# bywmm/RE-GNN

Measured on AMD Instinct MI355X. Metric: aggregated edges/sec per GPU (REGCN fwd+bwd, hidden=64); % HBM roofline, higher is better.
Workload: dtype fp32; 1 GPU; mag/regnn_ns.py REGCN neighbour-sampled train step: device sampler 512 papers/rank x fan-out [25, 20], group_input, 2x REGCNConv (hidden 64, mean, relation table, LN, ReLU, dropout 0.5), out_lin 349, nll, backward, Adam; mag_like(scale=10.0) replicated per rank; nodes=19397430, edges=422220140, relations=11, hidden=64, batch_per_rank=512, global_batch=512, parallelism=dp1, lookahead=16, hip_graph=True, engine=fused regnn_nsm_step

## Files before the change

### __graft_entry__.py

```python
import os
import sys

ROOT = os.path.dirname(os.path.abspath(__file__))
PKG = os.path.join(ROOT, "re-gnn_amd")
for _p in (ROOT, PKG):
    if _p not in sys.path:
        sys.path.insert(0, _p)


def build():
    from regnn_hip import build as b
    b.build()
    ob = os.path.join(ROOT, "oracle", "build_oracle.py")
    if os.path.exists(ob):
        import runpy
        runpy.run_path(ob, run_name="__main__")
    import layer
    import dgl
    from regnn_hip import _lib
    assert _lib.ABI_VERSION == 46


def smoke():
    import numpy as np
    import torch
    import torch.nn.functional as F

    build()
    sys.path.insert(0, os.path.join(ROOT, "tests"))
    import _golden as G
    from oracle import regnn_oracle as O
    import dgl
    from regnn_hip import nets

    d = G.load("model_regcn2")
    m = d["meta"]
    g = dgl.DGLGraph((d["g_src"], d["g_dst"]), num_nodes=int(d["g_N"])).to("cuda:0")
    net = nets.REGCN(g, int(d["g_R"]), m["alpha"], 64, 64, m["n_classes"], 2, F.elu, 0.0, m["dims"])
    P = G.sub(d, "p_", np.float32)
    with torch.no_grad():
        for n, p in net.named_parameters():
            p.copy_(torch.from_numpy(P[n]))
    net = net.to("cuda:0").eval()
    feats = [torch.from_numpy(d[f"feat{i}"]).to("cuda:0") for i in range(len(m["dims"]))]
    e_feat = torch.from_numpy(d["g_rel"]).to("cuda:0")
    logits, _ = net(feats, e_feat)
    logits.backward(torch.from_numpy(d["gout"]).to("cuda:0"))
    torch.cuda.synchronize()
    og = O.Graph(d["g_src"], d["g_dst"], int(d["g_N"]))
    ref_logits, _, ref_grads = O.regcn_model(
        og, [d[f"feat{i}"].astype(np.float64) for i in range(len(m["dims"]))], d["g_rel"],
        G.sub(d, "p_"), 2, m["alpha"], d["gout"].astype(np.float64))
    ok, err = G.close(logits.detach().cpu().numpy(), ref_logits, 1e-5)
# ... 10 lines not shown
```

### include/regnn_hip.h

```cpp
#ifndef REGNN_HIP_H
#define REGNN_HIP_H
#include <stdint.h>

#ifdef __cplusplus
extern "C" {
#endif

typedef struct ihipStream_t* hipStream_t;

enum { REGNN_OK = 0, REGNN_EINVAL = 1, REGNN_EUNSUPPORTED = 2, REGNN_ELAUNCH = 3 };
enum { REGNN_F32 = 0, REGNN_BF16 = 1 };
enum { REGNN_SELF_PRESCALED = 0x100 };

int regnn_abi_version(void);

int64_t regnn_tune(int32_t key, int64_t value);

int64_t regnn_slab_rows(int64_t n_seg, int32_t n_chunk);

int regnn_degree(const int32_t* ptr, const uint8_t* rel, const float* rel_table, int64_t n_seg,
                 float power, int32_t split, const int32_t* long_ids, int32_t n_long,
                 const int32_t* long_cnt, int32_t n_rel, float* deg, float* norm,
                 hipStream_t stream);

// ... 243 lines not shown
                   int32_t world, int64_t* state, int32_t* n_id, int32_t* sizes,
                   int64_t* stamp_src, hipStream_t stream);

#define REGNN_CSC_PIECE 1024
#define REGNN_CSC_LONG_CAP (32768 / 17 + 1)
#define REGNN_CSC_LONG_NPIECE (REGNN_CSC_LONG_CAP + 1)
#define REGNN_CSC_LONG_TAB (((REGNN_CSC_LONG_NPIECE + 1) + 3) / 4 * 4)
#define REGNN_CSC_LONG_MAXPIECE (32768 / REGNN_CSC_PIECE + REGNN_CSC_LONG_CAP)
#define REGNN_CSC_LONG_INTS (REGNN_CSC_LONG_TAB + 4 * REGNN_CSC_LONG_MAXPIECE)
int regnn_ns_hop(const int32_t* ptr, const int32_t* idx, const uint8_t* etype,
                 const int32_t* ntype, int32_t num_edge_types, int32_t k, int32_t hop,
                 int64_t* state, int32_t* sizes, int32_t* n_id, int32_t cap_dst,
                 uint64_t* g2l, uint64_t* first, int32_t* samp, int32_t* spos, int32_t* scnt,
                 int32_t* gsrc, uint8_t* flag, int32_t* tiles, uint64_t* status,
                 int32_t* blk_ptr, int32_t* blk_idx, uint8_t* blk_rel, int32_t* blk_pos,
                 int32_t* blk_row, float* inv, const int64_t* local, int32_t* edge_type,
                 int64_t* edge_off, int32_t meta_only, int32_t* csc_cnt, int32_t* csc_ptr,
                 int32_t* csc_ent, int32_t* csc_long, int32_t strided, hipStream_t stream);

typedef struct regnn_ns_csc_job {
    int32_t hop;
    int32_t cap_e;
    const int32_t* gsrc;
    const uint64_t* g2l;
    int32_t* blk_idx;
    const int32_t* blk_row;
    const uint8_t* blk_rel;
    int32_t* csc_cnt;
    int32_t* tiles;
    int32_t* csc_ptr;
    int32_t* csc_ent;
    int32_t* csc_long;
} regnn_ns_csc_job;
int regnn_ns_hop_typed_sums(const int32_t* ptr, const int32_t* idx, const uint8_t* etype,
                            const int32_t* ntype, int32_t num_edge_types, int32_t k, int32_t hop,
                            int64_t* state, int32_t* sizes, const int32_t* n_id, int32_t cap_dst,
                            int32_t* scnt, uint8_t* blk_rel, float* inv, const int64_t* local,
                            int32_t* edge_type, int64_t* edge_off, const float* const* tables,
                            int32_t n_types, int32_t K, float* s_agg, float* s_w, float* u_self,
                            int32_t* u_rel, const regnn_ns_csc_job* csc, hipStream_t stream);

int regnn_ns_spmm_bwd(const int32_t* ptr, const int32_t* idx, const uint8_t* rel,
                      const float* rel_table, const float* out_scale, const float* g,
                      const float* x, float* gx, float* slab, int32_t n_rel, int64_t n_rows,
                      int32_t F, hipStream_t stream);

int64_t regnn_ns_csc_hub_work_floats(int32_t F);
int regnn_ns_spmm_bwd_csc(const int32_t* csc_ptr, const int32_t* csc_ent, const int32_t* csc_long,
                          const float* rel_table, const float* out_scale, const float* g,
                          const float* x, float* gx, float* slab, int32_t n_rel,
                          const int32_t* sizes, int32_t size_idx, int64_t cap_rows, int32_t F,
                          int32_t slab_rows, float* hub_work, hipStream_t stream);

int regnn_ns_typed_agg(const int32_t* ptr, const int32_t* idx, const uint8_t* rel,
                       const float* rel_table, const int32_t* n_id, const int32_t* ntype,
                       const int64_t* local, const int32_t* e_type, const int64_t* e_off,
                       const float* const* tables, int32_t n_types, int32_t K, int64_t n_rows,
                       float* S, float* wsum, int64_t ld_s, int64_t ld_w, hipStream_t stream);

int regnn_ns_spmm_strided_fwd(const int32_t* live, const int32_t* cnt, int32_t stride,
                              const int32_t* idx, const uint8_t* rel, const float* rel_table,
                              const float* inv, const float* bias, const float* x, float* y,
                              int64_t n_rows, int32_t F, hipStream_t stream);

int regnn_ns_slot_agg(const int32_t* sizes, int32_t hop, const float* U, const float* cnt,
                      const float* x_self, const int32_t* u_rel, const float* rel_table,
                      int32_t n_et, int32_t n_types, int32_t K, int64_t cap, float* out,
                      int64_t ld, hipStream_t stream);
int regnn_ns_slot_agg_bwd(const int32_t* sizes, int32_t hop, const float* U, const float* cnt,
                          const float* x_self, const int32_t* u_rel, const float* g, int64_t ld,
                          int32_t n_et, int32_t n_types, int32_t K, float* slab, int32_t n_rel,
                          int32_t slab_rows, hipStream_t stream);

// ... 155 lines not shown
```

### re-gnn_amd/csrc/re_ns.hip

```cpp
#include "regnn_common.h"

#include <cstdlib>

namespace regnn {

constexpr int kNsTile = 1024;

__device__ __forceinline__ uint64_t mix64(uint64_t x) {
    x ^= x >> 30;
    x *= 0xBF58476D1CE4E5B9ull;
    x ^= x >> 27;
    x *= 0x94D049BB133111EBull;
    x ^= x >> 31;
    return x;
}

__device__ __forceinline__ uint64_t ns_hop_seed(const int64_t* state, int hop) {
    const uint64_t base = uint64_t(state[0]), epoch = uint64_t(state[1]),
                   batch = uint64_t(state[3]);
    return mix64(base ^ mix64((epoch << 40) ^ (batch << 8) ^ uint64_t(hop)));
}

__device__ __forceinline__ uint32_t ns_stamp(const int64_t* state, int hop) {
    return uint32_t(uint64_t(state[4]) * 8u + uint64_t(hop) + 1u);
// ... 755 lines not shown
        for (uint32_t spins = 0; spins < (1u << 26) && !seen; ++spins) {
            seen = uint32_t(__hip_atomic_load(ctl + 1, __ATOMIC_RELAXED,
                                              __HIP_MEMORY_SCOPE_AGENT)) == stamp;
            if (!seen) __builtin_amdgcn_s_sleep(1);
        }
        if (!seen) {
            __hip_atomic_store(ctl + 2, 1, __ATOMIC_RELAXED, __HIP_MEMORY_SCOPE_AGENT);
            ok = 0;
        }
        __builtin_amdgcn_fence(__ATOMIC_ACQUIRE, "agent");
        asm volatile("s_waitcnt vmcnt(0)" ::: "memory");
    }
    __syncthreads();
    if (lid >= 0 && ok) J.csc_ent[J.csc_ptr[lid] + rank] = ent;
}

inline int csc_blocks(int64_t cap_e) { return int((cap_e + kCscScanT - 1) / kCscScanT); }

__global__ void __launch_bounds__(kCscScanT)
ns_resolve_csc_kernel(NsCscJob J, const int32_t* __restrict__ sizes,
                      const int64_t* __restrict__ state) {
    csc_resolve_place<16>(J, sizes, state, blockIdx.x, gridDim.x);
}

struct NsSumArgs {
    const int32_t* ptr; const int32_t* idx; const uint8_t* etype; const int32_t* ntype;
    const int64_t* local; int n_et;
    const int32_t* n_id; int32_t* sizes; int hop; int cap; int k;
    int64_t* state;
    int32_t* scnt; uint8_t* blk_rel; float* inv; int32_t* e_type; int64_t* e_off;
    const float* xt[8]; int T;
    float* s_agg; float* s_w; float* u_self; int32_t* u_rel;
    NsCscJob csc; int csc_blocks;
};

template <int NT>
__device__ __forceinline__ const float* pick_tab(const NsSumArgs& A, int t) {
    const float* r = A.xt[0];
#pragma unroll
    for (int q = 1; q < NT; ++q)
        if (t == q) r = A.xt[q];
    return r;
}

constexpr int kNsSumK = 128;
#ifndef REGNN_NS_SUM_UN32
#define REGNN_NS_SUM_UN32 11
#endif
template <int G>
constexpr int ns_sum_un() { return G == 32 ? REGNN_NS_SUM_UN32 : 11; }
constexpr int kNsSumOcc = REGNN_NS_SUM_UN32 > 11 ? 3 : 4;
constexpr int kNsSumWaves = 4;

template <int G, int NT>
__global__ void __launch_bounds__(64 * kNsSumWaves, kNsSumOcc)
ns_sample_sums_kernel(NsSumArgs A) {
    if (int(blockIdx.x) < A.csc_blocks) {
        csc_resolve_place<4>(A.csc, A.sizes, A.state, blockIdx.x, A.csc_blocks);
        return;
    }
    const int bid = blockIdx.x - A.csc_blocks, nbk = gridDim.x - A.csc_blocks;
    constexpr int K = kNsSumK;
    constexpr int kNsSumUN = ns_sum_un<G>();
    constexpr int TPW = 64 / G;
    constexpr int H = G == 64 ? 2 : 1;
    __shared__ int wsum[kNsSumWaves * TPW];
    const int wl = threadIdx.x & 63, wv = threadIdx.x >> 6;
    const int lane = wl % G, tl = wv * TPW + wl / G;
    const uint64_t gmask = G == 64 ? ~0ull : (0xFFFFFFFFull << (wl & 32));
    const int n = A.sizes[A.hop];
    const int k = A.k, S = k + 1;
    int etot = 0;
    for (int ib = bid * (kNsSumWaves * TPW); ib < A.cap; ib += nbk * (kNsSumWaves * TPW)) {
    const int i = ib + tl;
    const int64_t base = int64_t(i) * S;
    int cnt = -1;
    if (i < A.cap && i >= n) {
        if (lane == 0) {
            A.scnt[i] = 0;
            A.inv[i] = 1.f;
        }
    } else if (i < n) {
        const uint64_t seed = ns_hop_seed(A.state, A.hop);
        const int t = A.n_id[i];
        const int b = A.ptr[t], d = A.ptr[t + 1] - b;
        cnt = d < k ? d : k;
        int slot = lane < d ? lane : -1, rank = lane;
        int src = lane;
        if (d > k) {
            slot = -1;
            const int jl = d - k + lane;
            const int my_pos = lane < k ? int((uint64_t(ns_hash(seed, uint64_t(t), uint64_t(jl))) *
                                               uint64_t(jl + 1)) >> 32) : 0;
            for (int q = 0; q < k; ++q) {
                const int pos = __shfl(my_pos, q, G);
                const bool seen = (__ballot(slot == pos) & gmask) != 0;
                if (lane == q) slot = seen ? d - k + q : pos;
            }
            rank = 0;
            for (int m = 0; m < k; ++m) {
                const int other = __shfl(slot, m, G);
                rank += (lane < k && other < slot) ? 1 : 0;
            }
            for (int m = 0; m < k; ++m)
                if (__shfl(rank, m, G) == lane) src = m;
        }
        int my_t = 0, my_lo = 0, my_r = 0;
        if (lane < cnt) {
            const int p = b + slot;
            const int u = A.idx[p];
            const int64_t bp = base + rank;
            my_r = A.etype[p];
            my_t = A.ntype[u];
            const int64_t lo = A.local[u];
            my_lo = int(lo);
            A.blk_rel[bp] = uint8_t(my_r);
            A.e_type[bp] = my_t;
            A.e_off[bp] = lo;
        }
        int st = __shfl(my_t, src, G), sr = __shfl(my_r, src, G), slo = __shfl(my_lo, src, G);
        if (lane == cnt) {
            const int64_t bp = base + cnt;
            st = A.ntype[t];
            sr = A.n_et + st;
            const int64_t lo = A.local[t];
            slo = int(lo);
            A.blk_rel[bp] = uint8_t(sr);
            A.e_type[bp] = st;
            A.e_off[bp] = lo;
        }
        if (lane == 0) {
            A.scnt[i] = cnt;
            A.inv[i] = 1.f / float(cnt + 1);
        }
        const int h = lane >> 5, l = lane & 31;
        const int ne = cnt + 1;
        float4 racc[NT];
        float ws[NT];
        int rt[NT];
#pragma unroll
        for (int tt = 0; tt < NT; ++tt) {
            racc[tt] = make_float4(0.f, 0.f, 0.f, 0.f);
            ws[tt] = 0.f;
            rt[tt] = -1;
        }
        float4 xs = make_float4(0.f, 0.f, 0.f, 0.f);
        int rs = -1;
        for (int j0 = 0; j0 < ne; j0 += H * kNsSumUN) {
            float4 x[kNsSumUN];
#pragma unroll
            for (int u = 0; u < kNsSumUN; ++u) {
                const int j = j0 + H * u + h;
                const int jj = j < ne ? j : ne - 1;
                const int tj = __shfl(st, jj, G);
                const int64_t lo = __shfl(slo, jj, G);
                x[u] = *reinterpret_cast<const float4*>(pick_tab<NT>(A, tj) + lo * K + 4 * l);
            }
#pragma unroll
            for (int u = 0; u < kNsSumUN; ++u) {
                const int j = j0 + H * u + h;
                const int jj = j < ne ? j : ne - 1;
                const int tj = __shfl(st, jj, G), rj = __shfl(sr, jj, G);
// ... 721 lines not shown
                       edge_type, edge_off, lean, csc_cnt, int(cap_e));
    REGNN_LAUNCH_CHECK();
    const int64_t slots = int64_t(cap_dst) * k;
    hipLaunchKernelGGL(ns_place_kernel, dim3(unsigned((slots + kBlock - 1) / kBlock)),
                       dim3(kBlock), 0, stream, samp, spos, scnt, sizes, hop, cap_dst, k, state,
                       etype, g2l, first, blk_ptr, blk_rel, blk_pos, blk_row, gsrc, ntype, local, edge_type,
                       edge_off, lean);
    REGNN_LAUNCH_CHECK();
    if (lean) return REGNN_OK;
    hipLaunchKernelGGL(ns_flags_kernel, dim3(n_tiles), dim3(kBlock), 0, stream, gsrc, sizes, hop,
                       state, g2l, first, flag, tiles, n_tiles, 0);
    REGNN_LAUNCH_CHECK();
    hipLaunchKernelGGL(ns_finish_kernel, dim3(n_tiles), dim3(kBlock), 0, stream, gsrc, sizes, hop,
                       state, flag, tiles, g2l, n_id, 0);
    REGNN_LAUNCH_CHECK();
    hipLaunchKernelGGL(ns_resolve_kernel, dim3(unsigned((cap_e + kBlock - 1) / kBlock)),
                       dim3(kBlock), 0, stream, gsrc, sizes, hop, g2l, blk_idx, int(cap_e), ntype, local,
                       edge_type, edge_off, csc_cnt, 0);
    REGNN_LAUNCH_CHECK();
    if (csc) {
        hipLaunchKernelGGL(ns_csc_kernel, dim3(1), dim3(kCscThreads), 0, stream, sizes, hop, blk_idx,
                           blk_row, blk_rel, csc_cnt, csc_ptr, csc_ent, csc_long, 0);
        REGNN_LAUNCH_CHECK();
    }
    return REGNN_OK;
}

int regnn_ns_hop_typed_sums(const int32_t* ptr, const int32_t* idx, const uint8_t* etype,
                            const int32_t* ntype, int32_t num_edge_types, int32_t k, int32_t hop,
                            int64_t* state, int32_t* sizes, const int32_t* n_id, int32_t cap_dst,
                            int32_t* scnt, uint8_t* blk_rel, float* inv, const int64_t* local,
                            int32_t* edge_type, int64_t* edge_off, const float* const* tables,
                            int32_t n_types, int32_t K, float* s_agg, float* s_w, float* u_self,
                            int32_t* u_rel, const regnn_ns_csc_job* csc, hipStream_t stream) {
    if (!ptr || !idx || !etype || !ntype || !state || !sizes || !n_id || !scnt || !blk_rel ||
        !inv || !local || !edge_type || !edge_off || !tables || !s_agg || !s_w || !u_self ||
        !u_rel || cap_dst <= 0 || hop < 0 || hop > 6 || num_edge_types < 0)
        return REGNN_EINVAL;
    if (K != kNsSumK || n_types < 1 || n_types > 4 || k < 1 || k > 63) return REGNN_EUNSUPPORTED;
    if (int64_t(cap_dst) * (k + 1) >= (int64_t(1) << 31)) return REGNN_EUNSUPPORTED;
    NsSumArgs A{};
    A.ptr = ptr; A.idx = idx; A.etype = etype; A.ntype = ntype; A.local = local;
    A.n_et = num_edge_types; A.n_id = n_id; A.sizes = sizes; A.hop = hop; A.cap = cap_dst;
    A.k = k; A.state = state; A.scnt = scnt; A.blk_rel = blk_rel; A.inv = inv;
    A.e_type = edge_type; A.e_off = edge_off; A.T = n_types;
    for (int t = 0; t < n_types; ++t) {
        if (!tables[t] || reinterpret_cast<uintptr_t>(tables[t]) % 16) return REGNN_EINVAL;
        A.xt[t] = tables[t];
    }
    for (int t = n_types; t < 8; ++t) A.xt[t] = tables[0];
    if (reinterpret_cast<uintptr_t>(s_agg) % 16 || reinterpret_cast<uintptr_t>(u_self) % 16)
        return REGNN_EINVAL;
    A.s_agg = s_agg; A.s_w = s_w; A.u_self = u_self; A.u_rel = u_rel;
    if (csc) {
        if (!csc->gsrc || !csc->g2l || !csc->blk_idx || !csc->blk_row || !csc->blk_rel ||
            !csc->csc_cnt || !csc->tiles || !csc->csc_ptr || !csc->csc_ent || !csc->csc_long ||
            csc->hop < 0 || csc->hop >= hop || csc->cap_e <= 0)
            return REGNN_EINVAL;
        if (csc->cap_e > kCscMax) return REGNN_EUNSUPPORTED;
        A.csc = NsCscJob{csc->hop, csc->cap_e, csc->gsrc, csc->g2l, csc->blk_idx, csc->blk_row,
                         csc->blk_rel, csc->csc_cnt, csc->tiles, csc->csc_ptr, csc->csc_ent,
                         csc->csc_long};
        A.csc_blocks = csc_blocks(csc->cap_e);
    }
    static const int sum_blocks = [] {
        const char* v = getenv("REGNN_NS_SUM_BLOCKS");
        return v ? atoi(v) : 0;
    }();
    auto grid = [&](int rows_per_block) {
        const int g = (cap_dst + rows_per_block - 1) / rows_per_block;
        return dim3(unsigned(A.csc_blocks + (sum_blocks > 0 && sum_blocks < g ? sum_blocks : g)));
    };
    if (k + 1 <= 32)
        hipLaunchKernelGGL((ns_sample_sums_kernel<32, 4>), grid(2 * kNsSumWaves),
                           dim3(64 * kNsSumWaves), 0, stream, A);
    else
        hipLaunchKernelGGL((ns_sample_sums_kernel<64, 4>), grid(kNsSumWaves),
                           dim3(64 * kNsSumWaves), 0, stream, A);
    REGNN_LAUNCH_CHECK();
    return REGNN_OK;
}

int regnn_ns_spmm_bwd(const int32_t* ptr, const int32_t* idx, const uint8_t* rel,
                      const float* rel_table, const float* out_scale, const float* g,
                      const float* x, float* gx, float* slab, int32_t n_rel, int64_t n_rows,
                      int32_t F, hipStream_t stream) {
    if (!ptr || !idx || !g || !gx || n_rows < 0 || F <= 0 || (F & 3) || n_rel < 0 ||
        n_rel > 256 || (slab && (!x || !rel || !rel_table || n_rel == 0)))
        return REGNN_EINVAL;
    if (n_rows == 0) return REGNN_OK;
    const int nvec = F / 4;
    int lpr = 16;
    while (nvec % lpr) lpr >>= 1;
    const int64_t rpb = int64_t(kBlock / 64) * (64 / lpr);
    int64_t grid = (n_rows + rpb - 1) / rpb;
    if (grid > kMaxGrid) grid = kMaxGrid;
    if (grid < 1) grid = 1;
#define NSB_CASE(L)                                                                            \
    if (lpr == L) {                                                                            \
        hipLaunchKernelGGL((ns_spmm_bwd_kernel<L>), dim3((unsigned)grid), dim3(kBlock), 0,     \
                           stream, ptr, idx, rel, rel_table, out_scale, g, x, gx, slab, n_rel, \
                           n_rows, F);                                                         \
        REGNN_LAUNCH_CHECK();                                                                  \
        return REGNN_OK;                                                                       \
    }
    NSB_CASE(16) NSB_CASE(8) NSB_CASE(4) NSB_CASE(2) NSB_CASE(1)
#undef NSB_CASE
    return REGNN_EUNSUPPORTED;
}

// ... 2 lines not shown
```

### re-gnn_amd/csrc/regnn_abi.hip

```cpp
#include "regnn_common.h"

extern "C" int regnn_abi_version(void) { return 46; }
```

### re-gnn_amd/regnn_hip/_lib.py

```python
import ctypes
import os

import torch

from .build import LIB

if not os.path.exists(LIB):
    raise ImportError(
        f"regnn_hip: native library {LIB} is missing — build it with "
        "`python -c 'import __graft_entry__ as g; g.build()'` (hipcc, gfx950). "
        "There is no CPU fallback.")

_so = ctypes.CDLL(os.environ.get("REGNN_LIB", LIB))

P = ctypes.c_void_p
I32 = ctypes.c_int32
I64 = ctypes.c_int64
U64 = ctypes.c_uint64
F32 = ctypes.c_float

_SIG = {
    "regnn_abi_version": ([], ctypes.c_int),
    "regnn_gemm_x6_work_floats": ([I64, I64, I32], I64),
    "regnn_copy2d_many": ([P, I32, P], ctypes.c_int),
# ... 41 lines not shown
    "regnn_gat_scores": ([P, P, P, P, P, P, I64, I32, F32, P, P], ctypes.c_int),
    "regnn_rel_reduce": ([P, I64, I32, P, I32, P], ctypes.c_int),
    "regnn_gat_softmax_fwd": ([P, P, P, P, P, P, I64, I32, F32, P, P, P], ctypes.c_int),
    "regnn_gat_softmax_bwd": ([P, P, P, P, P, P, P, P, I64, I32, F32, P, P, P, I32, P, P],
                              ctypes.c_int),
    "regnn_spmm_heads_fwd": ([P, P, P, P, P, P, I64, I32, I32, I32, P, P], ctypes.c_int),
    "regnn_gat_fused_fwd": ([P, P, P, P, P, P, P, P, P, I64, I32, I32, F32, I32, P, P, P],
                            ctypes.c_int),
    "regnn_gat_attn_lse": ([P, P, P, P, P, P, P, I64, I32, F32, P, P, P], ctypes.c_int),
    "regnn_spmm_heads_bwd": ([P, P, P, P, P, P, P, P, I64, I32, I32, I32, P, P], ctypes.c_int),
    "regnn_segment_sum": ([P, P, P, I64, I32, P, P, P], ctypes.c_int),
    "regnn_col_sum": ([P, I64, I32, P, P], ctypes.c_int),
    "regnn_type_project": ([P, I64, I32, I32, I32, P, P, P, P, ctypes.c_uint32, F32, I64, P, P, P],
                           ctypes.c_int),
    "regnn_linear_wgrad": ([P, I64, I32, I64, P, I32, I32, P, I32, P], ctypes.c_int),
    "regnn_row_scale": ([P, P, P, I64, I32, I32, P, ctypes.c_uint32, F32, P, P, P], ctypes.c_int),
    "regnn_softmax_xent": ([P, I64, I32, I64, P, F32, P, P, P], ctypes.c_int),
    "regnn_attn_dots_fwd": ([P, P, P, I64, I32, I32, P, P, P], ctypes.c_int),
    "regnn_attn_dots_bwd": ([P, P, P, P, P, I64, I32, I32, P, P, I32, P], ctypes.c_int),
    "regnn_head_fwd": ([P, I64, I32, P, P, I32, I64, P, I64, F32, P, P, P, P], ctypes.c_int),
    "regnn_sample_count": ([P, P, I64, I32, P, P], ctypes.c_int),
    "regnn_sample_fill": ([P, P, P, I64, I32, U64, P, P, P, P], ctypes.c_int),
    "regnn_ns_batch": ([P, I64, I32, I32, I32, P, P, P, P, P], ctypes.c_int),
    "regnn_ns_labels": ([P, P, P, I32, I64, P, P], ctypes.c_int),
    "regnn_rel_tab": ([P, P, I32, ctypes.c_float, ctypes.c_float, P, P], ctypes.c_int),
    "regnn_rel_tabs": ([P, P, P, P, I32, ctypes.c_float, ctypes.c_float, P], ctypes.c_int),
    "regnn_softmax_xent_fwd": ([P, P, I32, I32, I64, P, P, P, P], ctypes.c_int),
    "regnn_softmax_xent_bwd": ([P, P, P, P, P, I32, I32, I64, P, P], ctypes.c_int),
    "regnn_ns_xent_fwd": ([P, P, P, P, I32, I32, I64, P, P, P, P, P, P], ctypes.c_int),
    "regnn_xent_bwd_colsum": ([P, P, P, P, P, I32, I32, I64, P, P, P], ctypes.c_int),
    "regnn_ns_hop": ([P, P, P, P, I32, I32, I32, P, P, P, I32, P, P, P, P, P, P, P, P, P, P, P, P,
                      P, P, P, P, P, P, I32, P, P, P, P, I32, P], ctypes.c_int),
    "regnn_ns_hop_typed_sums": ([P, P, P, P, I32, I32, I32, P, P, P, I32, P, P, P, P, P, P, P,
                                 I32, I32, P, P, P, P, P, P], ctypes.c_int),
    "regnn_ns_spmm_bwd": ([P, P, P, P, P, P, P, P, P, I32, I64, I32, P], ctypes.c_int),
    "regnn_ns_csc_hub_work_floats": ([I32], I64),
    "regnn_ns_spmm_bwd_csc": ([P, P, P, P, P, P, P, P, P, I32, P, I32, I64, I32, I32, P, P],
                              ctypes.c_int),
    "regnn_ns_typed_agg": ([P, P, P, P, P, P, P, P, P, P, I32, I32, I64, P, P, I64, I64, P],
                           ctypes.c_int),
    "regnn_ns_typed_agg_bwd": ([P, P, P, P, P, P, P, P, P, I32, I32, I64, P, P, I64, I64, P, I32,
                                I32, P], ctypes.c_int),
    "regnn_ns_spmm_strided_fwd": ([P, P, I32, P, P, P, P, P, P, P, I64, I32, P], ctypes.c_int),
    "regnn_ns_slot_agg": ([P, I32, P, P, P, P, P, I32, I32, I32, I64, P, I64, P], ctypes.c_int),
    "regnn_ns_slot_agg_bwd": ([P, I32, P, P, P, P, P, I64, I32, I32, I32, P, I32, I32, P],
                              ctypes.c_int),
    "regnn_nsm_slab_floats": ([P, I32], I64),
    "regnn_nsm_step": ([P, P, P], ctypes.c_int),
    "regnn_adam_flat": ([P, P, P, P, I64, F32, F32, F32, F32, F32, F32, P, P, P], ctypes.c_int),
    "regnn_typed_gather": ([P, I64, P, P, I32, P, I32, P, P], ctypes.c_int),
    "regnn_typed_scatter": ([P, I64, P, P, I32, P, I32, P, P], ctypes.c_int),
    "regnn_typed_chunks": ([I64, I32, I32], I64),
    "regnn_typed_slab_floats": ([I64, I32, I32, I32], I64),
    "regnn_typed_linear_fwd": ([P, P, P, I64, I32, P, P, P, I32, I32, P, P], ctypes.c_int),
    "regnn_typed_linear_wgrad": ([P, P, P, I64, I32, P, P, I32, I32, I32, P, P, P, P, P],
                                 ctypes.c_int),
}

for _name, (_args, _ret) in _SIG.items():
    if os.environ.get("REGNN_LIB") and not hasattr(_so, _name):
        continue
    _f = getattr(_so, _name)
    _f.argtypes = _args
    _f.restype = _ret

EXPORTED = tuple(_SIG)
ABI_VERSION = 46
if _so.regnn_abi_version() != ABI_VERSION and not os.environ.get("REGNN_LIB"):
    raise ImportError(f"regnn_hip: ABI mismatch ({_so.regnn_abi_version()} != {ABI_VERSION}); "
                      "rebuild the library")

F32_CODE, BF16_CODE = 0, 1
SELF_PRESCALED = 0x100
_ERR = {1: "invalid argument", 2: "unsupported shape/dtype", 3: "kernel launch failed"}


def dtype_code(t):
    if t.dtype == torch.float32:
        return F32_CODE
    if t.dtype == torch.bfloat16:
        return BF16_CODE
    raise TypeError(f"regnn_hip: unsupported feature dtype {t.dtype} (float32 / bfloat16)")


class DevPtr(int):

    def __new__(cls, value, dev):
        o = int.__new__(cls, value)
        o.dev = dev
        return o


class _StreamArg:

    def __repr__(self):
        return "<regnn_hip current stream>"


_STREAM = _StreamArg()

# ... 40 lines not shown
```

### re-gnn_amd/regnn_hip/ns.py

```python
import ctypes
import os

import torch
import torch.nn.functional as F

from . import _lib as L
from .profile import enabled as profile_enabled, timed

M64 = (1 << 64) - 1


def _i64(u):
    u &= M64
    return u - (1 << 64) if u >= (1 << 63) else u


class NSBlock:

    is_ns_block = True

    def __init__(self, ptr, idx, rel, pos, inv, n_dst, n_src, E, device, row=None):
        self.csr_ptr, self.csr_idx, self.rel, self.pos, self.inv = ptr, idx, rel, pos, inv
        self.row = row
        self.n_dst, self.n_src, self.E = int(n_dst), int(n_src), int(E)
# ... 95 lines not shown
    def check_index(self):
        bad = self.index_errors().cpu().tolist()
        if any(bad):
            raise RuntimeError(f"regnn_ns_hop: the transposed index build timed out waiting for "
                               f"its publish (hops {[h for h, v in enumerate(bad) if v]})")

    def enable_csc(self, hop):
        ce = self.blocks[hop].csr_idx.numel()
        if ce > 32768:
            raise ValueError(f"the transposed index needs <= 32768 block edges, got {ce}")
        z = lambda n: torch.zeros(n, dtype=torch.int32, device=self.device)
        self.csc[hop] = (z(ce), z(ce + 1), z(ce), z(max(ce + 1, CSC_LONG_INTS)))
        return self.csc[hop]

    def batch_from_perm(self, perm, rank=0, world=1):
        L.call("regnn_ns_batch", L.ptr(perm), perm.numel(), self.B, int(rank), int(world),
               L.ptr(self.state), L.ptr(self.n_id), L.ptr(self.sizes),
               None if self.stamp_src is None else L.ptr(self.stamp_src), L.stream())

    def run_hops(self, meta_only=True, strided=None, csc_stream=None, before_sums=None):
        strided = self.strided if strided is None else bool(strided)
        hs = lambda h: strided if self.hop_strided[h] is None else self.hop_strided[h]
        rg = self.rg
        deferred = -1
        for h, k in enumerate(self.sizes_k):
            b, blk = self.hop_bufs[h], self.blocks[h]
            sh = hs(h)
            fork = (csc_stream is not None and sh and self.csc[h] is not None and
                    self.edge_meta[h] is None)
            if self._sums_path(h, sh, meta_only):
                if before_sums is not None:
                    before_sums()
                ts = self.typed_sums[h]
                et, eo = self.edge_meta[h]
                with timed("ns_typed_sums"):
                    L.call("regnn_ns_hop_typed_sums", L.ptr(rg.csr_ptr), L.ptr(rg.csr_idx),
                           L.ptr(self.etype_csr), L.ptr(self.ntype), self.num_edge_types, k, h,
                           L.ptr(self.state), L.ptr(self.sizes), L.ptr(self.n_id), self.caps[h],
                           L.ptr(b["scnt"]), L.ptr(blk.rel), L.ptr(blk.inv), L.ptr(self.local),
                           L.ptr(et), L.ptr(eo), ts["tables"], ts["T"], ts["K"],
                           L.ptr(ts["s_agg"]), L.ptr(ts["s_w"]), L.ptr(ts["u_self"]),
                           L.ptr(ts["u_rel"]),
                           ctypes.addressof(self._csc_job(h - 1)) if deferred == h - 1 else None,
                           L.stream())
                self.meta_fresh[h] = True
                self.sums_fresh[h] = True
                continue
            self.sums_fresh[h] = False
            defer = (not fork and sh and CSC_FUSE["mode"] != "off" and
                     self.csc[h] is not None and self.edge_meta[h] is None and
                     h + 1 < len(self.sizes_k) and self._sums_path(h + 1, hs(h + 1), meta_only))
            L.call("regnn_ns_hop", L.ptr(rg.csr_ptr), L.ptr(rg.csr_idx), L.ptr(self.etype_csr),
                   L.ptr(self.ntype), self.num_edge_types, k, h, L.ptr(self.state),
                   L.ptr(self.sizes), L.ptr(self.n_id), self.caps[h], L.ptr(self.g2l),
                   L.ptr(self.first), L.ptr(b["samp"]), L.ptr(b["spos"]), L.ptr(b["scnt"]),
                   L.ptr(b["gsrc"]), L.ptr(b["flag"]), L.ptr(b["tiles"]), L.ptr(b["status"]),
                   L.ptr(blk.csr_ptr),
                   L.ptr(blk.csr_idx), L.ptr(blk.rel), L.ptr(blk.pos), L.ptr(blk.row),
                   L.ptr(blk.inv),
                   *((L.ptr(self.local), L.ptr(self.edge_meta[h][0]), L.ptr(self.edge_meta[h][1]))
                     if self.edge_meta[h] is not None else (None, None, None)),
                   int(meta_only and self.meta_only[h] and self.edge_meta[h] is not None),
                   *((L.ptr(t) for t in self.csc[h]) if self.csc[h] is not None
                     else (None, None, None, None)),
                   2 if fork or defer else int(sh), L.stream())
            deferred = h if defer else -1
            if fork:
                csc_stream.wait_stream(torch.cuda.current_stream(self.device))
                with torch.cuda.stream(csc_stream):
                    self._hop_call(h, k, meta_only, 3)
            self.meta_fresh[h] = self.edge_meta[h] is not None
        self._csr_fresh = not strided

    def _sums_path(self, h, strided, meta_only):
        return (self.typed_sums[h] is not None and strided and meta_only and self.meta_only[h]
                and self.edge_meta[h] is not None)

    def _csc_job(self, h):
# ... 156 lines not shown
        return "inputs must be contiguous fp32"
    if model.out_lin.weight.shape[0] > 448 or model.out_lin.weight.shape[1] != 64:
        return "out_lin must be 64 -> <= 448"
    return None


REL_SLOTS = {"mode": "auto"}
STRIDED = {"mode": "on"}
FUSED_ADAM = {"mode": "on"}
SPLIT_JOIN = {"mode": os.environ.get("REGNN_NS_SPLIT_JOIN", "on")}
SPLIT_EXCHANGE = {"mode": os.environ.get("REGNN_NS_SPLIT_EXCHANGE", "off")}
MODULE_PIPELINE = {"mode": os.environ.get("REGNN_NS_MODULE_PIPELINE", "on")}
MODULE_AHEAD = {"n": int(os.environ.get("REGNN_NS_MODULE_AHEAD", "8"))}
LIN_XENT = {"mode": os.environ.get("REGNN_NS_LIN_XENT", "on")}
CSC_FORK = {"mode": os.environ.get("REGNN_NS_CSC_FORK", "off")}
CSC_FUSE = {"mode": os.environ.get("REGNN_NS_CSC_FUSE", "off")}
AHEAD = {"steps": int(os.environ["REGNN_NS_AHEAD"]) if "REGNN_NS_AHEAD" in os.environ else None}


def default_ahead(world):
    return AHEAD["steps"] if AHEAD["steps"] is not None else (16 if world == 1 else 8)
SUMS_ALIGN = {"mode": os.environ.get("REGNN_NS_SUMS_ALIGN", "2")}
GEMM_LIVE_HINT = {"mode": os.environ.get("REGNN_NS_GEMM_LIVE_HINT", "off")}
MODULE_PRE_SUMS = {"mode": os.environ.get("REGNN_NS_MODULE_PRESUMS", "on")}
MODULE_STRIDED = {"mode": os.environ.get("REGNN_NS_MODULE_STRIDED", "on")}
ADAM_PRE_STEP = {"mode": os.environ.get("REGNN_ADAM_PRE_STEP", "on")}
SAMPLER_LANES = {"n": int(os.environ.get("REGNN_NS_SAMPLER_LANES", "1"))}
MODULE_LEAN_HOP = {"mode": os.environ.get("REGNN_NS_MODULE_LEAN", "on")}
LEAN_LAST_HOP = {"mode": "on"}
PRE_SUMS = {"mode": os.environ.get("REGNN_NS_PRE_SUMS", "on")}
GROUP_ORDER = {"mode": os.environ.get("REGNN_NS_GROUP_ORDER", "model")}


def relation_slots_ok(sampler, T):
    rg = sampler.rg
    key = ("_regnn_rel_slots", sampler.num_edge_types, T)
    cache = getattr(rg, "_regnn_rel_slots", None)
    if cache is not None and cache[0] == key:
        return cache[1]
    dev = rg.device
    ptr = rg.csr_ptr.to(torch.int64)
    present = torch.zeros(_MT * _MT * 256, dtype=torch.bool, device=dev)
    step = 1 << 26
    for a in range(0, rg.E, step):
        b = min(rg.E, a + step)
        pos = torch.arange(a, b, device=dev)
        dst = torch.searchsorted(ptr, pos, right=True) - 1
        st = sampler.ntype[rg.csr_idx[a:b].to(torch.int64)].to(torch.int64)
        dt = sampler.ntype[dst].to(torch.int64)
        r = sampler.etype_csr[a:b].to(torch.int64)
        ok = (st >= 0) & (st < T) & (dt >= 0) & (dt < T)
        present[((dt * _MT + st) * 256 + r)[ok]] = True
    per_pair = present.view(_MT * _MT, 256).sum(1)
    ok = bool((per_pair <= 1).all().item())
    rg._regnn_rel_slots = (key, ok)
    return ok


class FusedStep:

    def __init__(self, model, sampler, x_dict, node_type, local_node_idx, y_flat, loss):
        why = fused_unsupported(model, x_dict)
        if why is not None:
            raise ValueError(f"regnn_nsm_step does not cover this model: {why}")
        dev = sampler.device
        self.device = dev
        nl = len(model.convs)
        if len(sampler.sizes_k) != nl:
            raise ValueError(f"{nl} layers need {nl} sampler hops, got {len(sampler.sizes_k)}")
        keys = sorted(x_dict)
        T, K = len(keys), int(x_dict[0].shape[1])
        C = int(model.out_lin.weight.shape[0])
        caps = sampler.caps
        self.keep = []

        def ptr(t):
            self.keep.append(t)
            return t.data_ptr()

        def grad_ptr(p):
            if p.grad is None:
                p_scratch = torch.zeros_like(p)
                return ptr(p_scratch)
            return ptr(p.grad)

        P = self.P = _NsmParams()
        P.n_types, P.k_in, P.n_layers, P.n_classes = T, K, nl, C
        P.alpha = float(model.convs[0].scaling_factor)
        P.p_drop = float(model.dropout) if model.training else 0.0
# ... 40 lines not shown
        W.s_w, W.beta = ptr(z(n0, T)), ptr(z(n0, T))
        W.nvalid = ptr(z(1))
        self.two_layer = (nl == 2 and C <= TWO_LAYER_MAX_CLASSES and
                          sampler.blocks[0].csr_idx.numel() <= 32768)
        P.two_layer = int(self.two_layer)
        if self.two_layer:
            W.p0 = ptr(z(caps[1], 64))
            W.gh1 = ptr(z(caps[0], 64))
            _, cptr, cent, clong = sampler.csc[0] or sampler.enable_csc(0)
            W.csc_ptr0, W.csc_ent0, W.csc_long0 = ptr(cptr), ptr(cent), ptr(clong)
            W.hub_acc = ptr(torch.zeros(_MAX_PIECE * 64, dtype=torch.int64, device=dev))
            W.hub_ticket = ptr(torch.zeros(_LONG_CAP, dtype=torch.int32, device=dev))
            W.hub_terms = ptr(torch.zeros(3 * 64 + 1, dtype=torch.int64, device=dev))
            sampler.strided = STRIDED["mode"] != "off"
            if sampler.strided:
                for h, k in enumerate(sampler.sizes_k):
                    W.stride[h] = k + 1
                    W.blk_cnt[h] = ptr(sampler.hop_bufs[h]["scnt"])
        self.adam = None
        P.n_edge_types = int(sampler.num_edge_types)
        P.rel_slots = int(REL_SLOTS["mode"] != "off" and relation_slots_ok(sampler, T))
        if P.rel_slots:
            W.u_self = ptr(z(n0, K))
            W.u_rel = ptr(torch.full((n0, T + 1), -1, dtype=torch.int32, device=dev))
        self.slab = z(_slab_floats(P, caps[0]))
        W.slab = ptr(self.slab)
        self.model, self.sampler, self.n_layers = model, sampler, nl
        if (PRE_SUMS["mode"] != "off" and self.two_layer and P.rel_slots and K == 128 and
                T <= 4 and sampler.strided and sampler.meta_only[nl - 1] and
                max(sampler.sizes_k) <= 63):
            self._tables = (ctypes.c_void_p * T)(*[x_dict[k].data_ptr() for k in keys])
            sampler.typed_sums[nl - 1] = dict(
                tables=self._tables, T=T, K=K, s_agg=self._buf(W.s_agg), s_w=self._buf(W.s_w),
                u_self=self._buf(W.u_self), u_rel=self._buf(W.u_rel))
            W.pre_sums = 1

    def _buf(self, addr):
        return next(t for t in self.keep if torch.is_tensor(t) and t.data_ptr() == addr)

    def attach_adam(self, opt, grad_flat):
        if not self.two_layer:
            raise ValueError("the fused optimizer needs the two-layer step")
        A = self.adam = _NsmAdam()
        A.param, A.exp_avg, A.exp_avg_sq = opt.p.data_ptr(), opt.m.data_ptr(), opt.v.data_ptr()
        A.grad_base, A.n = grad_flat.data_ptr(), grad_flat.numel()
        A.lr, A.beta1, A.beta2, A.eps = opt.lr, float(opt.betas[0]), float(opt.betas[1]), opt.eps
        A.weight_decay, A.grad_scale = opt.weight_decay, opt.grad_scale
        A.step, A.ticket = opt.step_count.data_ptr(), opt.ticket.data_ptr()
        self.keep.extend([opt.p, opt.m, opt.v, grad_flat, opt.step_count, opt.ticket])
        self.W.adam = ctypes.addressof(A)

    def kernels(self):
        if self.two_layer:
            ks = ["agg0", "head", "gather", "bwd0"] + ([] if self.P.rel_slots else ["rel0"])
            return ks + ["finalize+adam" if self.adam is not None else "finalize"]
        ks = ["prep", "agg0"] + ["agg"] * (self.n_layers - 2) + ["head"]
        ks += ["agg_bwd", "post_bwd"] * (self.n_layers - 1)
        ks += ["bwd0_rs" if self.P.rel_slots else "bwd0"]
        ks += [] if self.P.rel_slots else ["rel0"]
        return ks + ["finalize", "chain"]

    def launches(self):
        return len(self.kernels())

    def step(self, part=0):
        if part and not self.two_layer:
            raise ValueError("the step splits into parts only in its two-layer form")
        self.W.part = int(part)
        if part == 2:
            with torch.cuda.device(self.device):
                L.call("regnn_nsm_step", ctypes.addressof(self.P), ctypes.addressof(self.W),
                       torch.cuda.current_stream(self.device).cuda_stream)
            return
        if not self.sampler.meta_fresh[self.n_layers - 1]:
            raise RuntimeError("run the sampler's hops after building FusedStep: layer 0 reads the "
                               "per-edge source type / table row they write")
        if self.W.pre_sums and not self.sampler.sums_fresh[self.n_layers - 1]:
            raise RuntimeError("the sampler's latest batch did not form layer 0's input sums "
                               "(run_hops with meta_only=True and the strided layout, as the "
                               "fused step's sampling does)")
        self.P.p_drop = float(self.model.dropout) if self.model.training else 0.0
        with torch.cuda.device(self.device), timed("nsm_step"):
            L.call("regnn_nsm_step", ctypes.addressof(self.P), ctypes.addressof(self.W),
                   torch.cuda.current_stream(self.device).cuda_stream)


def group_sizes(ahead):
    out, m = [], int(ahead)
    while m >= 2:
        out.append(m)
        m //= 2
    return out


PLAN_ORDER = {"mode": os.environ.get("REGNN_NS_PLAN", "lead4")}


def _split(k, ahead):
    out = []
    while k > 0:
        m = next((m for m in group_sizes(ahead) if m <= k), 1)
        out.append(m)
        k -= m
    return out


def plan_sizes(k, ahead, order=None):
# ... 185 lines not shown
            last = len(s.sizes_k) - 1
            et, eo = s.enable_edge_meta(self.local_node_idx, last)
            s.meta_only[last] = True
            blk = s.blocks[last]
            blk.edge_meta, blk.meta_only = (et, eo), True
            self._module_pre_sums(s, last)
        for h, blk in enumerate(s.blocks):
            blk.live_rows = s.sizes[h:h + 1]
        if s.blocks[0].csr_idx.numel() <= 32768:
            _, cptr, cent, clong = s.csc[0] or s.enable_csc(0)
            b0 = s.blocks[0]
            b0.csc, b0.csc_cap = (cptr, cent, clong, s.sizes, 1), s.caps[1]
            from . import ops as _ops
            if (MODULE_STRIDED["mode"] != "off" and _ops.NS_CSC["mode"] != "off" and
                    len(s.sizes_k) > 1 and
                    getattr(self.model, "hidden_dim", 0) in _ops._CSC_WIDTHS):
                s.hop_strided[0] = True
                b0.strided_rows = (s.hop_bufs[0]["scnt"], s.sizes_k[0] + 1)

    def _module_pre_sums(self, s, last):
        tabs = getattr(self.model, "_type_tables", lambda _x: None)(self.x_dict)
        T = len(tabs) if tabs else 0
        if (MODULE_PRE_SUMS["mode"] == "off" or not tabs or T > 4 or
                any(t is None or t.dim() != 2 or t.shape[1] != 128 or not t.is_contiguous() or
                    t.data_ptr() % 16 for t in tabs) or max(s.sizes_k) > 63 or
                not relation_slots_ok(s, T)):
            return
        cap, K, dev = s.caps[last], 128, self.device
        z = lambda *shape: torch.zeros(*shape, dtype=torch.float32, device=dev)
        U, cnt, xself = z(cap, T, K), z(cap, T), z(cap, K)
        urel = torch.full((cap, T + 1), -1, dtype=torch.int32, device=dev)
        ptrs = (ctypes.c_void_p * T)(*[t.data_ptr() for t in tabs])
        s.typed_sums[last] = dict(tables=ptrs, T=T, K=K, s_agg=U, s_w=cnt, u_self=xself,
                                  u_rel=urel, keep=tabs)
        s.hop_strided[last] = True
        s.blocks[last].pre_sums = (U, cnt, xself, urel)

    def steps_per_epoch(self):
        nb = -(-self.train_idx.numel() // self.sampler.B)
        return -(-nb // self.world)

    def set_epoch(self, epoch):
        self.epoch = int(epoch)
        if self.shuffle:
            g = torch.Generator()
            g.manual_seed(self.seed * 1_000_003 + self.epoch)
            order = torch.randperm(self.train_idx.numel(), generator=g).to(self.device)
            self.perm.copy_(self.train_idx[order])
        else:
            self.perm.copy_(self.train_idx)
        for s in self.slots:
            st = s.state
            st[0:1].fill_(_i64(self.seed))
            st[1:2].fill_(self.epoch)
            st[2:3].zero_()
        self.cur, self._primed, self._trained = 0, False, 0

    @property
    def sampler(self):
        return self.slots[self._trained]

    def _sample(self, slot, before_sums=None):
        n = len(self.slots)
        s = self.slots[slot]
        s.batch_from_perm(self.perm, self.rank + slot * self.world, n * self.world)
        if self.fused is not None:
            csc = getattr(self, "_csc", None)
# ... 426 lines not shown
```

Before: 1.118 billion edges/s.

## Derive node type, local row and relation arithmetically in typed-sums sampler

When node types are laid out contiguously and each (dst type, src type) pair maps to a single relation, the typed-sums sampling kernel computes source type, local offset and relation from type offset boundaries and a packed pair table. This replaces gathers from the ntype, local and etype arrays. It also skips writing the per-edge metadata (blk_rel, e_type, e_off) when the fused step does not read it, and caps the grid at the number of resident blocks. The price is a one-time host-side layout check, plus the assumption that the relation is fully determined by the type pair.

```diff
diff --git a/__graft_entry__.py b/__graft_entry__.py
--- a/__graft_entry__.py
+++ b/__graft_entry__.py
@@ -18,7 +18,7 @@
     import layer
     import dgl
     from regnn_hip import _lib
-    assert _lib.ABI_VERSION == 46
+    assert _lib.ABI_VERSION == 47
 
 
 def smoke():
diff --git a/include/regnn_hip.h b/include/regnn_hip.h
--- a/include/regnn_hip.h
+++ b/include/regnn_hip.h
@@ -299,13 +299,19 @@
     int32_t* csc_ent;
     int32_t* csc_long;
 } regnn_ns_csc_job;
+typedef struct regnn_ns_type_layout {
+    int32_t n_types;
+    int64_t type_off[5];
+    int32_t pair_rel[4][4];
+} regnn_ns_type_layout;
 int regnn_ns_hop_typed_sums(const int32_t* ptr, const int32_t* idx, const uint8_t* etype,
                             const int32_t* ntype, int32_t num_edge_types, int32_t k, int32_t hop,
                             int64_t* state, int32_t* sizes, const int32_t* n_id, int32_t cap_dst,
                             int32_t* scnt, uint8_t* blk_rel, float* inv, const int64_t* local,
                             int32_t* edge_type, int64_t* edge_off, const float* const* tables,
                             int32_t n_types, int32_t K, float* s_agg, float* s_w, float* u_self,
-                            int32_t* u_rel, const regnn_ns_csc_job* csc, hipStream_t stream);
+                            int32_t* u_rel, const regnn_ns_csc_job* csc,
+                            const regnn_ns_type_layout* layout, hipStream_t stream);
 
 int regnn_ns_spmm_bwd(const int32_t* ptr, const int32_t* idx, const uint8_t* rel,
                       const float* rel_table, const float* out_scale, const float* g,
diff --git a/re-gnn_amd/csrc/re_ns.hip b/re-gnn_amd/csrc/re_ns.hip
--- a/re-gnn_amd/csrc/re_ns.hip
+++ b/re-gnn_amd/csrc/re_ns.hip
@@ -811,7 +811,20 @@
     const float* xt[8]; int T;
     float* s_agg; float* s_w; float* u_self; int32_t* u_rel;
     NsCscJob csc; int csc_blocks;
+    int toff[4]; uint32_t pair[4];
 };
+
+__device__ __forceinline__ int ns_type_of(const NsSumArgs& A, int u) {
+    return (u >= A.toff[1] ? 1 : 0) + (u >= A.toff[2] ? 1 : 0) + (u >= A.toff[3] ? 1 : 0);
+}
+
+__device__ __forceinline__ int ns_type_first(const NsSumArgs& A, int t) {
+    int o = 0;
+#pragma unroll
+    for (int q = 1; q < 4; ++q)
+        if (t == q) o = A.toff[q];
+    return o;
+}
 
 template <int NT>
 __device__ __forceinline__ const float* pick_tab(const NsSumArgs& A, int t) {
@@ -831,7 +844,7 @@
 constexpr int kNsSumOcc = REGNN_NS_SUM_UN32 > 11 ? 3 : 4;
 constexpr int kNsSumWaves = 4;
 
-template <int G, int NT>
+template <int G, int NT, bool DERIVE>
 __global__ void __launch_bounds__(64 * kNsSumWaves, kNsSumOcc)
 ns_sample_sums_kernel(NsSumArgs A) {
     if (int(blockIdx.x) < A.csc_blocks) {
@@ -885,28 +898,57 @@
                 if (__shfl(rank, m, G) == lane) src = m;
         }
         int my_t = 0, my_lo = 0, my_r = 0;
+        const bool meta = A.blk_rel != nullptr;
+        int tt0 = 0;
+        uint32_t pw = 0;
+        if constexpr (DERIVE) {
+            tt0 = ns_type_of(A, t);
+            pw = A.pair[0];
+#pragma unroll
+            for (int q = 1; q < 4; ++q)
+                if (tt0 == q) pw = A.pair[q];
+        }
         if (lane < cnt) {
             const int p = b + slot;
             const int u = A.idx[p];
             const int64_t bp = base + rank;
-            my_r = A.etype[p];
-            my_t = A.ntype[u];
-            const int64_t lo = A.local[u];
-            my_lo = int(lo);
-            A.blk_rel[bp] = uint8_t(my_r);
-            A.e_type[bp] = my_t;
-            A.e_off[bp] = lo;
+            int64_t lo;
+            if constexpr (DERIVE) {
+                my_t = ns_type_of(A, u);
+                my_lo = u - ns_type_first(A, my_t);
+                my_r = int((pw >> (8 * my_t)) & 0xFFu);
+                lo = my_lo;
+            } else {
+                my_r = A.etype[p];
+                my_t = A.ntype[u];
+                lo = A.local[u];
+                my_lo = int(lo);
+            }
+            if (meta) {
+                A.blk_rel[bp] = uint8_t(my_r);
+                A.e_type[bp] = my_t;
+                A.e_off[bp] = lo;
+            }
         }
         int st = __shfl(my_t, src, G), sr = __shfl(my_r, src, G), slo = __shfl(my_lo, src, G);
         if (lane == cnt) {
             const int64_t bp = base + cnt;
-            st = A.ntype[t];
+            int64_t lo;
+            if constexpr (DERIVE) {
+                st = tt0;
+                slo = t - ns_type_first(A, tt0);
+                lo = slo;
+            } else {
+                st = A.ntype[t];
+                lo = A.local[t];
+                slo = int(lo);
+            }
             sr = A.n_et + st;
-            const int64_t lo = A.local[t];
-            slo = int(lo);
-            A.blk_rel[bp] = uint8_t(sr);
-            A.e_type[bp] = st;
-            A.e_off[bp] = lo;
+            if (meta) {
+                A.blk_rel[bp] = uint8_t(sr);
+                A.e_type[bp] = st;
+                A.e_off[bp] = lo;
+            }
         }
         if (lane == 0) {
             A.scnt[i] = cnt;
@@ -1694,11 +1736,31 @@
                             int32_t* scnt, uint8_t* blk_rel, float* inv, const int64_t* local,
                             int32_t* edge_type, int64_t* edge_off, const float* const* tables,
                             int32_t n_types, int32_t K, float* s_agg, float* s_w, float* u_self,
-                            int32_t* u_rel, const regnn_ns_csc_job* csc, hipStream_t stream) {
-    if (!ptr || !idx || !etype || !ntype || !state || !sizes || !n_id || !scnt || !blk_rel ||
-        !inv || !local || !edge_type || !edge_off || !tables || !s_agg || !s_w || !u_self ||
-        !u_rel || cap_dst <= 0 || hop < 0 || hop > 6 || num_edge_types < 0)
+                            int32_t* u_rel, const regnn_ns_csc_job* csc,
+                            const regnn_ns_type_layout* layout, hipStream_t stream) {
+    if (!ptr || !idx || !state || !sizes || !n_id || !scnt || !inv || !tables || !s_agg ||
+        !s_w || !u_self || !u_rel || cap_dst <= 0 || hop < 0 || hop > 6 || num_edge_types < 0)
         return REGNN_EINVAL;
+    if (!layout && (!etype || !ntype || !local)) return REGNN_EINVAL;
+    if ((blk_rel || edge_type || edge_off) && !(blk_rel && edge_type && edge_off))
+        return REGNN_EINVAL;
+    int toff[4] = {0, INT32_MAX, INT32_MAX, INT32_MAX};
+    uint32_t pair[4] = {~0u, ~0u, ~0u, ~0u};
+    if (layout) {
+        if (layout->n_types != n_types || n_types < 1 || n_types > 4 || layout->type_off[0] != 0)
+            return REGNN_EINVAL;
+        for (int t = 0; t < n_types; ++t)
+            if (layout->type_off[t + 1] < layout->type_off[t]) return REGNN_EINVAL;
+        for (int a = 0; a < n_types; ++a)
+            for (int b = 0; b < n_types; ++b) {
+                const int r = layout->pair_rel[a][b];
+                if (r < -1 || r >= num_edge_types) return REGNN_EINVAL;
+                if (r > 254) return REGNN_EUNSUPPORTED;
+                if (r >= 0) pair[a] = (pair[a] & ~(0xFFu << (8 * b))) | (uint32_t(r) << (8 * b));
+            }
+        if (layout->type_off[n_types] >= INT32_MAX) return REGNN_EUNSUPPORTED;
+        for (int t = 1; t < n_types; ++t) toff[t] = int(layout->type_off[t]);
+    }
     if (K != kNsSumK || n_types < 1 || n_types > 4 || k < 1 || k > 63) return REGNN_EUNSUPPORTED;
     if (int64_t(cap_dst) * (k + 1) >= (int64_t(1) << 31)) return REGNN_EUNSUPPORTED;
     NsSumArgs A{};
@@ -1706,6 +1768,10 @@
     A.n_et = num_edge_types; A.n_id = n_id; A.sizes = sizes; A.hop = hop; A.cap = cap_dst;
     A.k = k; A.state = state; A.scnt = scnt; A.blk_rel = blk_rel; A.inv = inv;
     A.e_type = edge_type; A.e_off = edge_off; A.T = n_types;
+    for (int q = 0; q < 4; ++q) {
+        A.toff[q] = toff[q];
+        A.pair[q] = pair[q];
+    }
     for (int t = 0; t < n_types; ++t) {
         if (!tables[t] || reinterpret_cast<uintptr_t>(tables[t]) % 16) return REGNN_EINVAL;
         A.xt[t] = tables[t];
@@ -1729,15 +1795,37 @@
         const char* v = getenv("REGNN_NS_SUM_BLOCKS");
         return v ? atoi(v) : 0;
     }();
+    static const int resident = [] {
+        int dev = 0, n_cu = 0;
+        if (hipGetDevice(&dev) != hipSuccess ||
+            hipDeviceGetAttribute(&n_cu, hipDeviceAttributeMultiprocessorCount, dev) != hipSuccess ||
+            n_cu <= 0)
+            n_cu = 256;
+        return n_cu * (4 * kNsSumOcc / kNsSumWaves);
+    }();
     auto grid = [&](int rows_per_block) {
         const int g = (cap_dst + rows_per_block - 1) / rows_per_block;
-        return dim3(unsigned(A.csc_blocks + (sum_blocks > 0 && sum_blocks < g ? sum_blocks : g)));
+        int nb = g;
+        if (sum_blocks > 0) {
+            nb = sum_blocks < g ? sum_blocks : g;
+        } else if (sum_blocks == 0 && g > resident) {
+            const int rounds = (g + resident - 1) / resident;
+            nb = (g + rounds - 1) / rounds;
+        }
+        return dim3(unsigned(A.csc_blocks + nb));
     };
-    if (k + 1 <= 32)
-        hipLaunchKernelGGL((ns_sample_sums_kernel<32, 4>), grid(2 * kNsSumWaves),
+    const bool derive = layout != nullptr;
+    if (k + 1 <= 32 && derive)
+        hipLaunchKernelGGL((ns_sample_sums_kernel<32, 4, true>), grid(2 * kNsSumWaves),
+                           dim3(64 * kNsSumWaves), 0, stream, A);
+    else if (k + 1 <= 32)
+        hipLaunchKernelGGL((ns_sample_sums_kernel<32, 4, false>), grid(2 * kNsSumWaves),
+                           dim3(64 * kNsSumWaves), 0, stream, A);
+    else if (derive)
+        hipLaunchKernelGGL((ns_sample_sums_kernel<64, 4, true>), grid(kNsSumWaves),
                            dim3(64 * kNsSumWaves), 0, stream, A);
     else
-        hipLaunchKernelGGL((ns_sample_sums_kernel<64, 4>), grid(kNsSumWaves),
+        hipLaunchKernelGGL((ns_sample_sums_kernel<64, 4, false>), grid(kNsSumWaves),
                            dim3(64 * kNsSumWaves), 0, stream, A);
     REGNN_LAUNCH_CHECK();
     return REGNN_OK;
diff --git a/re-gnn_amd/csrc/regnn_abi.hip b/re-gnn_amd/csrc/regnn_abi.hip
--- a/re-gnn_amd/csrc/regnn_abi.hip
+++ b/re-gnn_amd/csrc/regnn_abi.hip
@@ -1,3 +1,3 @@
 #include "regnn_common.h"
 
-extern "C" int regnn_abi_version(void) { return 46; }
+extern "C" int regnn_abi_version(void) { return 47; }
diff --git a/re-gnn_amd/regnn_hip/_lib.py b/re-gnn_amd/regnn_hip/_lib.py
--- a/re-gnn_amd/regnn_hip/_lib.py
+++ b/re-gnn_amd/regnn_hip/_lib.py
@@ -97,7 +97,7 @@
     "regnn_ns_hop": ([P, P, P, P, I32, I32, I32, P, P, P, I32, P, P, P, P, P, P, P, P, P, P, P, P,
                       P, P, P, P, P, P, I32, P, P, P, P, I32, P], ctypes.c_int),
     "regnn_ns_hop_typed_sums": ([P, P, P, P, I32, I32, I32, P, P, P, I32, P, P, P, P, P, P, P,
-                                 I32, I32, P, P, P, P, P, P], ctypes.c_int),
+                                 I32, I32, P, P, P, P, P, P, P], ctypes.c_int),
     "regnn_ns_spmm_bwd": ([P, P, P, P, P, P, P, P, P, I32, I64, I32, P], ctypes.c_int),
     "regnn_ns_csc_hub_work_floats": ([I32], I64),
     "regnn_ns_spmm_bwd_csc": ([P, P, P, P, P, P, P, P, P, I32, P, I32, I64, I32, I32, P, P],
@@ -130,7 +130,7 @@
     _f.restype = _ret
 
 EXPORTED = tuple(_SIG)
-ABI_VERSION = 46
+ABI_VERSION = 47
 if _so.regnn_abi_version() != ABI_VERSION and not os.environ.get("REGNN_LIB"):
     raise ImportError(f"regnn_hip: ABI mismatch ({_so.regnn_abi_version()} != {ABI_VERSION}); "
                       "rebuild the library")
diff --git a/re-gnn_amd/regnn_hip/ns.py b/re-gnn_amd/regnn_hip/ns.py
--- a/re-gnn_amd/regnn_hip/ns.py
+++ b/re-gnn_amd/regnn_hip/ns.py
@@ -151,18 +151,22 @@
                 if before_sums is not None:
                     before_sums()
                 ts = self.typed_sums[h]
-                et, eo = self.edge_meta[h]
+                lay = ts.get("layout")
+                mode = SUMS_META["mode"]
+                skip = (lay is not None and ts.get("meta_unread", False) and mode != "on" and
+                        (mode == "off" or torch.cuda.is_current_stream_capturing()))
+                rel, et, eo = (None, None, None) if skip else (blk.rel, *self.edge_meta[h])
                 with timed("ns_typed_sums"):
                     L.call("regnn_ns_hop_typed_sums", L.ptr(rg.csr_ptr), L.ptr(rg.csr_idx),
                            L.ptr(self.etype_csr), L.ptr(self.ntype), self.num_edge_types, k, h,
                            L.ptr(self.state), L.ptr(self.sizes), L.ptr(self.n_id), self.caps[h],
-                           L.ptr(b["scnt"]), L.ptr(blk.rel), L.ptr(blk.inv), L.ptr(self.local),
+                           L.ptr(b["scnt"]), L.ptr(rel), L.ptr(blk.inv), L.ptr(self.local),
                            L.ptr(et), L.ptr(eo), ts["tables"], ts["T"], ts["K"],
                            L.ptr(ts["s_agg"]), L.ptr(ts["s_w"]), L.ptr(ts["u_self"]),
                            L.ptr(ts["u_rel"]),
                            ctypes.addressof(self._csc_job(h - 1)) if deferred == h - 1 else None,
-                           L.stream())
-                self.meta_fresh[h] = True
+                           None if lay is None else ctypes.addressof(lay), L.stream())
+                self.meta_fresh[h] = not skip
                 self.sums_fresh[h] = True
                 continue
             self.sums_fresh[h] = False
@@ -385,29 +389,98 @@
 GROUP_ORDER = {"mode": os.environ.get("REGNN_NS_GROUP_ORDER", "model")}
 
 
-def relation_slots_ok(sampler, T):
+TYPE_LAYOUT = {"mode": os.environ.get("REGNN_NS_TYPE_LAYOUT", "on")}
+SUMS_META = {"mode": os.environ.get("REGNN_NS_SUMS_META", "auto")}
+
+
+def pair_relations(node_type, csr_ptr, csr_idx, etype_csr, T):
+    dev = csr_ptr.device
+    ptr = csr_ptr.to(torch.int64)
+    E = int(csr_idx.numel())
+    present = torch.zeros(_MT * _MT * 256, dtype=torch.bool, device=dev)
+    step = 1 << 26
+    for a in range(0, E, step):
+        b = min(E, a + step)
+        pos = torch.arange(a, b, device=dev)
+        dst = torch.searchsorted(ptr, pos, right=True) - 1
+        st = node_type[csr_idx[a:b].to(torch.int64)].to(torch.int64)
+        dt = node_type[dst].to(torch.int64)
+        r = etype_csr[a:b].to(torch.int64)
+        ok = (st >= 0) & (st < T) & (dt >= 0) & (dt < T)
+        present[((dt * _MT + st) * 256 + r)[ok]] = True
+    present = present.view(_MT, _MT, 256)[:T, :T]
+    per_pair = present.sum(2)
+    single = bool((per_pair <= 1).all().item())
+    rel = torch.where(per_pair == 1, present.to(torch.float32).argmax(2),
+                      torch.full_like(per_pair, -1))
+    return rel.cpu(), single
+
+
+def _pair_table(sampler, T):
     rg = sampler.rg
     key = ("_regnn_rel_slots", sampler.num_edge_types, T)
     cache = getattr(rg, "_regnn_rel_slots", None)
-    if cache is not None and cache[0] == key:
-        return cache[1]
-    dev = rg.device
-    ptr = rg.csr_ptr.to(torch.int64)
-    present = torch.zeros(_MT * _MT * 256, dtype=torch.bool, device=dev)
-    step = 1 << 26
-    for a in range(0, rg.E, step):
-        b = min(rg.E, a + step)
-        pos = torch.arange(a, b, device=dev)
-        dst = torch.searchsorted(ptr, pos, right=True) - 1
-        st = sampler.ntype[rg.csr_idx[a:b].to(torch.int64)].to(torch.int64)
-        dt = sampler.ntype[dst].to(torch.int64)
-        r = sampler.etype_csr[a:b].to(torch.int64)
-        ok = (st >= 0) & (st < T) & (dt >= 0) & (dt < T)
-        present[((dt * _MT + st) * 256 + r)[ok]] = True
-    per_pair = present.view(_MT * _MT, 256).sum(1)
-    ok = bool((per_pair <= 1).all().item())
-    rg._regnn_rel_slots = (key, ok)
-    return ok
+    if cache is None or cache[0] != key:
+        rel, ok = pair_relations(sampler.ntype, rg.csr_ptr, rg.csr_idx, sampler.etype_csr, T)
+        cache = rg._regnn_rel_slots = (key, ok, rel)
+    return cache
+
+
+def relation_slots_ok(sampler, T):
+    return _pair_table(sampler, T)[1]
+
+
+def type_layout(node_type, local_node_idx, csr_ptr, csr_idx, etype_csr, T, pairs=None):
+    if T < 1 or T > 4:
+        return None
+    nt = node_type.reshape(-1).to(torch.int64)
+    lo = local_node_idx.reshape(-1).to(torch.int64)
+    n = int(nt.numel())
+    if n == 0 or lo.numel() != n or n >= 2 ** 31 - 1:
+        return None
+    if int(nt.min()) < 0 or int(nt.max()) >= T or bool((nt[1:] < nt[:-1]).any()):
+        return None
+    off = torch.zeros(T + 1, dtype=torch.int64, device=nt.device)
+    off[1:] = torch.cumsum(torch.bincount(nt, minlength=T), 0)
+    if not bool((lo == torch.arange(n, device=nt.device) - off[nt]).all()):
+        return None
+    rel, single = pairs if pairs is not None else pair_relations(nt, csr_ptr, csr_idx,
+                                                                 etype_csr, T)
+    if not single:
+        return None
+    return dict(T=T, type_off=[int(v) for v in off.cpu().tolist()],
+                pair_rel=[[int(v) for v in row] for row in rel.tolist()])
+
+
+class _NsTypeLayout(ctypes.Structure):
+    _fields_ = [("n_types", ctypes.c_int32), ("type_off", ctypes.c_int64 * 5),
+                ("pair_rel", (ctypes.c_int32 * 4) * 4)]
+
+
+def layout_struct(lay):
+    s = _NsTypeLayout()
+    s.n_types = lay["T"]
+    for t, v in enumerate(lay["type_off"]):
+        s.type_off[t] = v
+    for a in range(4):
+        for b in range(4):
+            s.pair_rel[a][b] = lay["pair_rel"][a][b] if a < lay["T"] and b < lay["T"] else -1
+    return s
+
+
+def sampler_type_layout(sampler, T):
+    if TYPE_LAYOUT["mode"] == "off" or sampler.local is None:
+        return None
+    rg = sampler.rg
+    key = ("_regnn_type_layout", sampler.num_edge_types, T, sampler.local.data_ptr())
+    cache = getattr(rg, "_regnn_type_layout", None)
+    if cache is None or cache[0] != key:
+        _, ok, rel = _pair_table(sampler, T)
+        lay = type_layout(sampler.ntype, sampler.local, rg.csr_ptr, rg.csr_idx,
+                          sampler.etype_csr, T, pairs=(rel, ok))
+        cache = rg._regnn_type_layout = (key, None if lay is None else layout_struct(lay),
+                                         sampler.local)
+    return cache[1]
 
 
 class FusedStep:
@@ -514,7 +587,8 @@
             self._tables = (ctypes.c_void_p * T)(*[x_dict[k].data_ptr() for k in keys])
             sampler.typed_sums[nl - 1] = dict(
                 tables=self._tables, T=T, K=K, s_agg=self._buf(W.s_agg), s_w=self._buf(W.s_w),
-                u_self=self._buf(W.u_self), u_rel=self._buf(W.u_rel))
+                u_self=self._buf(W.u_self), u_rel=self._buf(W.u_rel),
+                layout=sampler_type_layout(sampler, T), meta_unread=True)
             W.pre_sums = 1
 
     def _buf(self, addr):
@@ -554,7 +628,7 @@
                 L.call("regnn_nsm_step", ctypes.addressof(self.P), ctypes.addressof(self.W),
                        torch.cuda.current_stream(self.device).cuda_stream)
             return
-        if not self.sampler.meta_fresh[self.n_layers - 1]:
+        if not self.W.pre_sums and not self.sampler.meta_fresh[self.n_layers - 1]:
             raise RuntimeError("run the sampler's hops after building FusedStep: layer 0 reads the "
                                "per-edge source type / table row they write")
         if self.W.pre_sums and not self.sampler.sums_fresh[self.n_layers - 1]:
@@ -806,7 +880,8 @@
         urel = torch.full((cap, T + 1), -1, dtype=torch.int32, device=dev)
         ptrs = (ctypes.c_void_p * T)(*[t.data_ptr() for t in tabs])
         s.typed_sums[last] = dict(tables=ptrs, T=T, K=K, s_agg=U, s_w=cnt, u_self=xself,
-                                  u_rel=urel, keep=tabs)
+                                  u_rel=urel, keep=tabs,
+                                  layout=sampler_type_layout(s, T), meta_unread=True)
         s.hop_strided[last] = True
         s.blocks[last].pre_sums = (U, cnt, xself, urel)
 
```

Result: faster. 1.184 billion edges/s (median of 6 runs) (+5.9%).
